# nauful/NLZM

Hardware: AMD Instinct MI355X
Metric: compress MB/s (higher is better)
Workload: dtype u8; 1 GPU; enwik9 stand-in: 1000000000 B stream, -window:28; step = 41 launches of 8 chunks (40136704 B) of the stream; timed: bytes [200683520, 401367040) of 1000000000 (a prefix: the steps asked for end before the stream does); window_bits=28, batch_chunks=8, whole_stream=False

## Files before the change

### nlzm_amd/csrc/nlzm_hip.cpp

```cpp
#include <hip/hip_runtime.h>
#include <dirent.h>
#include <unistd.h>

#include <stdarg.h>
#include <stdint.h>
#include <stdio.h>
#include <stdlib.h>
#include <string.h>

#include <mutex>
#include <vector>

#include "nlzm_host_state.h"
#include "nlzm_report.h"

#include "nlzm_launch.h"

using namespace nlzm;
using namespace nlzm::host;

namespace {

char g_err[kErrText] = "";
std::mutex g_err_mu;
char *thread_err() { return t_dev ? t_dev->err : nullptr; }

int g_hwq_effective = 0;

inline uint32_t clampu(uint32_t v, uint32_t lo, uint32_t hi) { return v < lo ? lo : (v > hi ? hi : v); }

}

namespace nlzm {
int host_error(int code, const char *text)
{
    std::lock_guard<std::mutex> lk(g_err_mu);
    snprintf(g_err, sizeof g_err, "%s", text);
    if (char *te = thread_err()) memcpy(te, g_err, sizeof g_err);
    return code;
}
namespace host {

void error_prefixed(char (&out)[kErrText], const char *text, const char *prefix_fmt, ...)
{
    char prefix[32];
    va_list ap;
    va_start(ap, prefix_fmt);
    vsnprintf(prefix, sizeof prefix, prefix_fmt, ap);
    va_end(ap);
    std::lock_guard<std::mutex> lk(g_err_mu);
    snprintf(out, sizeof out, "%s%.*s", prefix, (int)sizeof out - 32, text ? text : g_err);
}
void error_replace(const char (&text)[kErrText])
{
    std::lock_guard<std::mutex> lk(g_err_mu);
    memcpy(g_err, text, sizeof g_err);
}

DevState g_dev0;
thread_local DevState *t_dev = nullptr;

void free_stream_buffers(Ctx &C)
{
    for (void *p : C.owned) (void)hipFree(p);
    C.owned.clear();
    C.buf = StreamBuffers{}; C.set[0] = C.set[1] = LaunchSet{}; C.set_idx = 0;
    C.open = false;
}
void release_own_io(Ctx &C)
{
    if (C.own_in) { (void)hipFree(C.own_in); C.own_in = nullptr; }
    if (C.own_dst) { (void)hipFree(C.own_dst); C.own_dst = nullptr; }
}
int alloc_own_io(Ctx &C, uint64_t n, uint64_t bound)
{
    release_own_io(C);
    HIPCHK(hipMalloc(&C.own_in, n + 512));
    HIPCHK(hipMalloc(&C.own_dst, bound));
    HIPCHK(hipMemsetAsync(C.own_in + n, 0, 512, C.st));
    return 0;
}

void make_geom(uint64_t n, uint32_t hist_bits_req, Geom &g)
{
    uint32_t hb = hist_bits_req;
    while (hb > 10 && n < (1ull << (hb - 1))) --hb;
    g.n = n;
    g.wbits = hb; g.wmask = (1u << hb) - 1;
    g.frame_bits = clampu(hb - 2, 14, 17);
    g.frame_size = 1u << g.frame_bits;
    g.chunk_size = ((g.frame_size * 15) / 16) - 0x200;
    g.feed = g.chunk_size + kMatchMax + 1;
    g.ht3_shift = 32 - (12 + clampu(hb, 15, 17) - 15);
    g.bt_shift = 32 - (13 + clampu(hb, 16, 20) - 16);
    g.rk_shift = 32 - (15 + clampu(hb, 16, 22) - 16);
    g.tag_mask = (uint32_t)((1ull << (32 - hb)) - 1);
    g.nchunks = (uint32_t)((n + g.chunk_size - 1) / g.chunk_size);
    g.bt_tmask = g.wmask;
}

// ... 2 lines not shown
    uint32_t tb = clampu(g.wbits + 5, 16, 33);
    uint32_t lgn = 1; while ((1ull << lgn) < g.n) lgn++;
    const uint32_t want = lgn + (uint32_t)tbits_per;
    if (want < tb) tb = want < 16 ? 16 : want;
    if ((int64_t)tb > tbits_max) tb = (uint32_t)(tbits_max < 16 ? 16 : tbits_max);
    return tb;
}
bool prefilter_is_bitmap(const Geom &g) { return g.n <= (unsigned long long)g.wmask + 1; }
size_t prefilter_bytes(uint32_t t_bits, bool bitmap)
{
    return bitmap ? (((size_t)1 << t_bits) / 8 < 4 ? (size_t)4 : ((size_t)1 << t_bits) / 8) : (size_t)4 << t_bits;
}
double launch_bytes_per_chunk(const Geom &g) { return 2300.0 * g.chunk_size + 8.0 * g.chunk_size * 4; }

namespace {
int alloc_launch_set(Ctx &C, LaunchSet &S)
{
    const StreamConfig &K = C.cfg;
    const unsigned long long bpos = (unsigned long long)K.batch * C.g.chunk_size;
    DEVALLOC(S.rkhash, K.rkhash_len * 4 + 16);
    DEVALLOC(S.syms, K.batch * K.syms_stride * 4);
    DEVALLOC(S.bits, K.batch * K.bits_stride);
    DEVALLOC(S.fmeta, K.batch * sizeof(FrameMeta));
    DEVALLOC(S.unc, bpos + 16);
    DEVALLOC(S.bt_ready, bpos * 4 * kBtRec);
    DEVALLOC(S.bt_flag, bpos * 4);
    DEVALLOC(S.abort_word, 4);
    DEVALLOC(S.bin_off, (size_t)K.batch * (K.nheads + 1) * 4);
    DEVALLOC(S.bin_pos, bpos * 8);
    if (K.hot_max) {
        DEVALLOC(S.hot_of_bin, (size_t)K.nheads * 4);
        DEVALLOC(S.hot_list, ((size_t)K.hot_max + 1) * 4);
    }
    if (K.in_set) DEVALLOC(S.snap, sizeof(v2::RoundSnap));
    return 0;
}
}

int stream_begin(Ctx &C, const Options &O, const void *d_src, uint64_t n, uint32_t hist_bits_req, void *d_dst, uint64_t dst_cap)
{
    if (!C.inited) return fail(NLZM_HIP_E_NODEVICE, "nlzm_hip_init() has not succeeded");
    if (n >= 0xFFFF0000ull) return fail(NLZM_HIP_E_TOOBIG, "input of %llu bytes needs >32-bit positions", (unsigned long long)n);
    if (hist_bits_req < 10 || hist_bits_req > 28) return fail(NLZM_HIP_E_ARG, "hist_bits %u outside [10,28]", hist_bits_req);
    if (dst_cap < 8) return fail(NLZM_HIP_E_CAPACITY, "dst_cap < 8");
    free_stream_buffers(C);
    make_geom(n, hist_bits_req, C.g);
    const Geom &g = C.g;
    C.d_in = (const uint8_t *)d_src; C.d_dst = (uint8_t *)d_dst; C.dst_cap = dst_cap;
    C.out_pos = 0; C.next_chunk = 0; C.pre_chunk = 0; C.last_launch_ms = 0;
    memset(&C.stats, 0, sizeof C.stats);
    memset(&C.tm, 0, sizeof C.tm);
    C.stats.in_bytes = n;
    StreamConfig &K = C.cfg;
    StreamBuffers &B = C.buf;
    K = StreamConfig{};
    K.in_set = C.pool != nullptr;
    K.batch = (uint32_t)(O.batch < 1 ? 1 : O.batch);
    if (g.nchunks && K.batch > g.nchunks) K.batch = g.nchunks;
    {
        const int64_t room = (int64_t)C.cu_count - (int64_t)pipeline2_role_blocks();
        if (room < 1) return fail(NLZM_HIP_E_ARG, "device has %d CUs: the pipeline needs at least %u", C.cu_count, pipeline2_role_blocks() + 1);
        K.worker_blocks = (uint32_t)(O.worker_blocks > room ? room : (O.worker_blocks < 1 ? 1 : O.worker_blocks));
    }
    K.worker_threads = (uint32_t)O.worker_threads;
    {
        K.nheads = 1u << (32 - g.bt_shift);
        const unsigned long long lanes = (unsigned long long)K.worker_blocks * K.worker_threads;
// ... 12 lines not shown
    K.syms_stride = 3ull * g.chunk_size + 4096;
    K.bits_stride = 2ull * g.chunk_size + 64;
    K.frame_stride = 12 + K.bits_stride + 16 + 2 * K.syms_stride;

    const size_t ht3_bytes = (size_t)8 << (32 - g.ht3_shift), rk_bytes = (size_t)4 << (32 - g.rk_shift), heads_bytes = (size_t)4 << (32 - g.bt_shift);
    {
        const unsigned long long need = (1ull << g.wbits) + (unsigned long long)K.batch * g.chunk_size;
        unsigned long long slots = 1ull << g.wbits;
        while (slots < need) slots <<= 1;
        C.g.bt_tmask = (uint32_t)(slots - 1);
    }
    const size_t tree_bytes = ((size_t)g.bt_tmask + 1) * 8;
    DEVALLOC(B.ht2, 4096 * 4);
    DEVALLOC(B.ht3, ht3_bytes);
    DEVALLOC(B.rk_table, rk_bytes);
    DEVALLOC(B.bt_heads, heads_bytes);
    DEVALLOC(B.bt_tree, tree_bytes);
    DEVALLOC(B.persist, sizeof(Persist));
    DEVFILL(hipMemsetAsync(B.ht2, 0xFF, 4096 * 4, C.st));
    DEVFILL(hipMemsetAsync(B.ht3, 0xFF, ht3_bytes, C.st));
    DEVFILL(hipMemsetAsync(B.rk_table, 0xFF, rk_bytes, C.st));
    DEVFILL(hipMemsetAsync(B.bt_heads, 0xFF, heads_bytes, C.st));
    DEVFILL(hipMemsetAsync(B.bt_tree, 0xFF, tree_bytes, C.st));

    Persist P;
    memset(&P, 0, sizeof P);
    for (uint32_t ctx = 0; ctx < kNumCtx; ctx++) {
        const uint32_t ns = (ctx == kCtxCmd) ? 4 : ((ctx == kCtxLenDirect || ctx >= kCtxSlotHi) ? 8 : 16);
        for (uint32_t i = 0; i <= ns; i++) P.cdf[ctx * kCdfStride + i] = (uint16_t)(i * (16384 / ns));
    }
    for (int i = 0; i < 4; i++) P.rep[i] = (uint32_t)i + 1;
    DEVFILL(hipMemcpyAsync(B.persist, &P, sizeof P, hipMemcpyHostToDevice, C.st));

    if (!K.in_set) {
        size_t free_b = 0, total_b = 0;
        HIPCHK(hipMemGetInfo(&free_b, &total_b));
        const double room = 0.6 * (double)free_b - 4.0 * (double)(1ull << K.t_bits);
        const double per_chunk = launch_bytes_per_chunk(g);
        if (room > per_chunk && (double)K.batch * per_chunk > room) K.batch = (uint32_t)(room / per_chunk);
    }
    const unsigned long long bpos = (unsigned long long)K.batch * g.chunk_size;
    K.rkhash_len = bpos + g.feed + 256 + 1024 + 2048;
    if (K.rkhash_len > n + 2048) K.rkhash_len = n + 2048;
    { uint32_t lg = 1; while ((1ull << lg) < bpos) lg++; K.m_bits = lg + 6 > 28 ? 28 : lg + 6; }
    K.ext_cap = K.pstride < kBtMaxPairs ? (uint32_t)(bpos / 64 + 1024) : 0u;
    if (K.ext_cap && O.block_ext_blocks >= 0) K.ext_cap = (uint32_t)(O.block_ext_blocks < 1 ? 1 : O.block_ext_blocks);

    DEVALLOC(B.scratch, K.batch * K.syms_stride * 4);
    DEVALLOC(B.frames, K.batch * K.frame_stride);
    DEVALLOC(B.dst_off, K.batch * sizeof(unsigned long long));
    for (uint32_t s = 0; s < (K.in_set ? 2u : 1u); s++) { const int rc = alloc_launch_set(C, C.set[s]); if (rc) return rc; }

    for (;;) {
        const int rc_t = dev_alloc(C, &B.pf_T, prefilter_bytes(K.t_bits, K.t_bitmap != 0));
        if (!rc_t) break;
        if (K.in_set || rc_t != NLZM_HIP_E_NOMEM || K.t_bits <= 28) return rc_t;
        (void)hipGetLastError();
        K.t_bits--;
    }
    DEVALLOC(B.pf_M, (size_t)4 << K.m_bits);
    DEVFILL(hipMemsetAsync(B.pf_T, 0, prefilter_bytes(K.t_bits, K.t_bitmap != 0), C.st));
    DEVFILL(hipMemsetAsync(B.pf_M, 0xFF, (size_t)4 << K.m_bits, C.st));
    DEVALLOC(B.pf_h, bpos * 4);
    DEVALLOC(B.pf_h2, bpos * 4);
    DEVALLOC(B.pf_c1, bpos);
    DEVALLOC(B.bt_pairs, bpos * (2ull * K.pstride * 4));
    if (K.ext_cap) DEVALLOC(B.bt_ext, (size_t)K.ext_cap * (2ull * (kBtMaxPairs - K.pstride) * 4));
    DEVALLOC(B.bin_cur, (size_t)K.batch * K.nheads * 4);
    DEVALLOC(B.wcnt, sizeof(WorkerCounters));
    DEVFILL(hipMemsetAsync(B.wcnt, 0, sizeof(WorkerCounters), C.st));
    DEVALLOC(B.bt_undo, (size_t)K.nheads * worker_undo_bytes_per_lane());
    if (K.hot_max) DEVALLOC(B.hot_undo, (size_t)K.hot_max * worker_hot_undo_bytes_per_wave());

    DEVALLOC(B.v2_ft, (size_t)v2::kFtRing * v2::kFtStride * 4);
    DEVALLOC(B.v2_tp, (size_t)v2::kTpRing * v2::kTpStride * 4);
    DEVALLOC(B.v2_tf, (size_t)v2::kTpRing * v2::kTfStride * 4);
    DEVALLOC(B.v2_state, sizeof(v2::StateV2));
    DEVALLOC(B.v2_hx, sizeof(v2::Hx));
    if (K.helper) DEVALLOC(B.v2_hb, v2::kHelpers * sizeof(v2::HelpBox));
    DEVFILL(hipMemsetAsync(B.v2_state, 0, sizeof(v2::StateV2), C.st));
    C.v2_launch_no = 0;

    const uint8_t hdr[4] = { (uint8_t)(g.wbits >> 8), (uint8_t)g.wbits, (uint8_t)(g.frame_bits >> 8), (uint8_t)g.frame_bits };
    DEVFILL(hipMemcpyAsync(C.d_dst, hdr, 4, hipMemcpyHostToDevice, C.st));
    C.out_pos = 4;

    if (C.pool && C.pool->measuring) return 0;
    HIPCHK(hipStreamSynchronize(C.st));
    C.open = true;
    return 0;
}

int step_pre(Ctx &C, uint32_t todo, StepPlan &P, bool ahead)
{
    const Geom &g = C.g;
    const StreamConfig &K = C.cfg;
    const StreamBuffers &B = C.buf;
    if (ahead) { if (!K.in_set) return fail(NLZM_HIP_E_ARG, "no second launch set"); C.set_idx ^= 1; }
    const LaunchSet &L = C.set[C.set_idx];
    const uint32_t c0 = C.pre_chunk, nb = todo < K.batch ? todo : K.batch, c1 = c0 + nb;
    C.pre_chunk = c1;
    P.c0 = c0; P.c1 = c1; P.nb = nb;
    P.set = C.set_idx; P.ahead = ahead;
    hipEvent_t *ev = C.ev[P.set];
    Globals &G = P.G;
    memset(&G, 0, sizeof G);
    G.in = C.d_in; G.rkhash = nullptr; G.ht2 = B.ht2; G.ht3 = B.ht3; G.rk_table = B.rk_table;
    G.bt_heads = B.bt_heads; G.bt_tree = B.bt_tree; G.persist = B.persist;
    G.syms = L.syms; G.syms_stride = K.syms_stride; G.bits = L.bits; G.bits_stride = K.bits_stride;
    G.fmeta = L.fmeta; G.chunk0 = c0;
    G.cap_words = C.stage.cap_words; G.cap_cap = C.stage.cap_cap; G.cap_lo = C.stage.cap_lo; G.cap_hi = C.stage.cap_hi; G.cap_used = C.stage.cap_used;
    G.workers = 1;
    const unsigned long long a0 = (unsigned long long)c0 * g.chunk_size;
    unsigned long long a1 = (unsigned long long)c1 * g.chunk_size;
    if (a1 > g.n) a1 = g.n;
    G.batch_a0 = (uint32_t)a0;
    {
        const unsigned long long lo = a0 > 1024 ? a0 - 1024 : 0;
        unsigned long long hi = a1 + g.feed + 256;
        if (hi + 255 > g.n) hi = g.n >= 255 ? g.n - 255 : 0;
        HIPCHK(hipEventRecord(ev[kEvRkBegin], C.st));
        if (hi > lo && hi - lo > K.rkhash_len) return fail(NLZM_HIP_E_ARG, "launch of %u chunks is larger than the stream was opened for", nb);
        G.rkhash = L.rkhash - lo;
        if (g.n >= 256 && hi > lo) launch_rk_hash(C.d_in, g.n, lo, hi, L.rkhash - lo, C.st);
    }
    HIPCHK(hipEventRecord(ev[kEvRkEnd], C.st));
    {
        const unsigned long long cnt = a1 - a0;
        G.bt_ready = L.bt_ready; G.bt_pairs = B.bt_pairs; G.bt_flag = L.bt_flag; G.unc = L.unc;
        G.bt_pstride = K.pstride; G.bt_ext = B.bt_ext; G.bt_ext_cap = K.ext_cap; G.bt_ext_cur = &B.v2_hx->ext_cur;
        G.bin_off = L.bin_off; G.bin_pos = L.bin_pos; G.nheads = K.nheads; G.wthreads = K.worker_threads;
        G.abort_word = L.abort_word; G.wcnt = B.wcnt; G.bt_undo = B.bt_undo;
        HIPCHK(hipMemsetAsync(L.bt_ready, 0, cnt * 4 * kBtRec, C.st));
        HIPCHK(hipMemsetAsync(L.bt_flag, 0, cnt * 4, C.st));
        HIPCHK(hipMemsetAsync(L.abort_word, 0, 4, C.st));
        HIPCHK(hipMemsetAsync(L.bin_off, 0, (size_t)nb * (K.nheads + 1) * 4, C.st));
        launch_prefilter(C.d_in, g.n, (uint32_t)a0, (uint32_t)a1, g.wmask, K.t_bits, K.t_bitmap, K.m_bits, B.pf_T, B.pf_M, B.pf_h, B.pf_h2,
                         B.pf_c1, L.unc, C.st);
        launch_bin(C.d_in, g, c0, nb, K.nheads, L.bin_off, B.bin_cur, L.bin_pos, L.unc, (uint32_t)a0, C.st);
        if (K.hot_max) {
            const unsigned long long lpos = (unsigned long long)K.batch * g.chunk_size;
            const double by_pace = K.in_set ? (double)lpos / 480.0 : (C.last_launch_ms > 0 ? 24.0 * C.last_launch_ms : (double)lpos / 240.0);
            const uint32_t hot_min = K.hot_min > 0 ? K.hot_min : (uint32_t)(by_pace < 512 ? 512 : (by_pace > 1e9 ? 1e9 : by_pace));
            launch_hot_select(L.bin_off, nb, K.nheads, K.hot_max, hot_min, L.hot_of_bin, L.hot_list, B.wcnt, C.st);
            G.hot_of_bin = L.hot_of_bin; G.hot_list = L.hot_list; G.hot_undo = B.hot_undo;
        }
    }
    {
        v2::Hx &h = C.hx_host;
        memset(&h, 0, sizeof h);
        h.f_pos = h.t_pos = h.t_out = h.p_pos = (uint32_t)a0;
        h.p_seg = ((unsigned long long)(uint32_t)a0 << 32) | (uint32_t)a0;
        if (!ahead) HIPCHK(hipMemcpyAsync(B.v2_hx, &h, sizeof h, hipMemcpyHostToDevice, C.st));
        P.V.ft = B.v2_ft; P.V.tp = B.v2_tp; P.V.tf = B.v2_tf; P.V.hx = B.v2_hx; P.V.state = B.v2_state; P.V.hb = B.v2_hb;
        G.progress = &B.v2_hx->f_pos;
        G.test_fail = K.test_fail_launch >= 0 && (int64_t)C.v2_launch_no == K.test_fail_launch ? 1u : 0u;
        G.table_shape = K.table_shape; G.launch_par = (uint32_t)(C.v2_launch_no++ & 1u);
    }
    HIPCHK(hipEventRecord(ev[kEvPrepEnd], C.st));
    return 0;
}

int step_post_issue(Ctx &C, const StepPlan &P)
{
    const StreamConfig &K = C.cfg;
    const LaunchSet &L = C.set[P.set];
    hipEvent_t *ev = C.ev[P.set];
    const uint32_t nb = P.nb;
    C.post_hm.resize(nb); C.post_hoff.resize(nb);
    C.post_aborted = 0;
    HIPCHK(hipEventRecord(ev[kEvLaunchEnd], C.st));
    launch_rans(L.syms, K.syms_stride, L.bits, K.bits_stride, L.fmeta, C.buf.scratch, K.syms_stride, C.buf.frames,
                K.frame_stride, (uint32_t)K.frame_stride, nb, C.st);
    HIPCHK(hipEventRecord(ev[kEvCoderEnd], C.st));
    HIPCHK(hipMemcpyAsync(C.post_hm.data(), L.fmeta, nb * sizeof(FrameMeta), hipMemcpyDeviceToHost, C.st));
    if (P.ahead) {
        HIPCHK(hipMemcpyAsync(&C.post_snap, L.snap, sizeof(v2::RoundSnap), hipMemcpyDeviceToHost, C.st));
        return 0;
    }
    HIPCHK(hipMemcpyAsync(&C.post_P, C.buf.persist, sizeof C.post_P, hipMemcpyDeviceToHost, C.st));
    HIPCHK(hipMemcpyAsync(&C.post_aborted, L.abort_word, 4, hipMemcpyDeviceToHost, C.st));
    HIPCHK(hipMemcpyAsync(&C.hx_host, C.buf.v2_hx, sizeof(v2::Hx), hipMemcpyDeviceToHost, C.st));
    return 0;
}
int step_post_check(Ctx &C, const StepPlan &P)
{
    const Geom &g = C.g;
    const StreamConfig &K = C.cfg;
    const LaunchSet &L = C.set[P.set];
    hipEvent_t *ev = C.ev[P.set];
    const uint32_t c0 = P.c0, c1 = P.c1, nb = P.nb;
    std::vector<FrameMeta> &hm = C.post_hm;
    std::vector<unsigned long long> &hoff = C.post_hoff;
    HIPCHK(hipStreamSynchronize(C.st));
    HIPCHK(hipGetLastError());
    if (P.ahead) { C.post_P.error = C.post_snap.error; C.post_P.next_chunk = C.post_snap.next_chunk; C.post_aborted = C.post_snap.aborted; C.hx_host = C.post_snap.hx; }
    const Persist &Pst = C.post_P;
    const uint32_t aborted = C.post_aborted;
    float rk_ms = 0, pre_ms = 0;
    HIPCHK(hipEventElapsedTime(&rk_ms, ev[kEvRkBegin], ev[kEvRkEnd]));
    HIPCHK(hipEventElapsedTime(&pre_ms, ev[kEvRkEnd], ev[kEvPrepEnd]));
    C.tm.prep_ms += rk_ms + pre_ms; C.tm.prep_launches += 5; C.tm.total_ms += rk_ms + pre_ms;
    C.arena_out = false;
    if (Pst.error || C.hx_host.err) {
        const v2::Hx &h = C.hx_host;
        WorkerCounters wc{};
        (void)hipMemcpy(&wc, C.buf.wcnt, sizeof wc, hipMemcpyDeviceToHost);
        char where[kErrText];
        stage_error_text(where, sizeof where, h, wc);
        return fail(NLZM_HIP_E_KERNEL, "device error %u in chunks [%u,%u) (parser stopped at chunk %u): %s", Pst.error ? Pst.error : h.err, c0, c1, Pst.next_chunk, where);
    }
    C.arena_out = K.ext_cap && C.hx_host.ext_cur > K.ext_cap;
    if (C.arena_out) return fail(NLZM_HIP_E_KERNEL, "the extension arena of the BT4 pair lists (%u blocks per launch) was used up in chunks [%u,%u): more positions with over %u "
                                     "record-setters than a block set reserves for", K.ext_cap, c0, c1, K.pstride);
    if (aborted) return fail(NLZM_HIP_E_KERNEL, "worker lanes aborted (code %u) in chunks [%u,%u)", aborted, c0, c1);
    if (Pst.next_chunk != c1) return fail(NLZM_HIP_E_KERNEL, "master stopped at chunk %u, expected %u", Pst.next_chunk, c1);
    unsigned long long pos = C.out_pos;
    for (uint32_t f = 0; f < nb; f++) {
        const uint32_t room = g.frame_size - ((c0 + f) == 0 ? 4 : 0);
        if (hm[f].out_len > room)
            return fail(NLZM_HIP_E_KERNEL, "frame %u is %u bytes: the reference would assert (:610)", c0 + f, hm[f].out_len);
        hoff[f] = pos; pos += hm[f].out_len;
    }
    if (pos + 4 > C.dst_cap) return fail(NLZM_HIP_E_CAPACITY, "dst_cap %llu too small", (unsigned long long)C.dst_cap);
    if (StageCapture &S = C.stage; S.want_frame >= (int64_t)c0 && S.want_frame < (int64_t)c1) {
        const uint32_t f = (uint32_t)(S.want_frame - c0);
        S.got_meta = hm[f];
        S.got_syms.resize(hm[f].nsyms); S.got_bits.resize(hm[f].nbits_bytes);
        HIPCHK(hipMemcpy(S.got_syms.data(), L.syms + f * K.syms_stride, hm[f].nsyms * 4ull, hipMemcpyDeviceToHost));
        HIPCHK(hipMemcpy(S.got_bits.data(), L.bits + f * K.bits_stride, hm[f].nbits_bytes, hipMemcpyDeviceToHost));
        S.got = true;
    }
    HIPCHK(hipMemcpyAsync(C.buf.dst_off, hoff.data(), nb * sizeof(unsigned long long), hipMemcpyHostToDevice, C.st));
    HIPCHK(hipEventRecord(ev[kEvGatherBegin], C.st));
    launch_gather(C.buf.frames, K.frame_stride, C.buf.dst_off, L.fmeta, C.d_dst, nb, C.st);
    HIPCHK(hipEventRecord(ev[kEvGatherEnd], C.st));
    C.post_pos = pos;
    return 0;
}
int step_post_done(Ctx &C, const StepPlan &P, float pipe_ms)
{
    hipEvent_t *ev = C.ev[P.set];
    const unsigned long long pos = C.post_pos;
    const uint32_t c1 = P.c1;
    HIPCHK(hipStreamSynchronize(C.st));
    float a = pipe_ms, b = 0, c = 0;
    if (pipe_ms < 0) HIPCHK(hipEventElapsedTime(&a, ev[kEvLaunchBegin], ev[kEvLaunchEnd]));
    HIPCHK(hipEventElapsedTime(&b, ev[kEvLaunchEnd], ev[kEvCoderEnd]));
    HIPCHK(hipEventElapsedTime(&c, ev[kEvGatherBegin], ev[kEvGatherEnd]));
    C.tm.match_parse_ms += a; C.tm.match_parse_launches++;
    if (a > 0) C.last_launch_ms = a;
    C.tm.rans_ms += b + c; C.tm.rans_launches++;
    C.tm.total_ms += a + b + c;
    C.out_pos = pos;
    C.next_chunk = c1;
    return 0;
}
namespace {
int step_post(Ctx &C, const StepPlan &P, float pipe_ms)
{
    int rc = step_post_issue(C, P);
    if (!rc) rc = step_post_check(C, P);
    if (!rc) rc = step_post_done(C, P, pipe_ms);
    return rc;
}
}

int stream_step(Ctx &C, uint32_t max_chunks, uint64_t *in_done, uint64_t *out_done, int *finished)
{
    if (!C.open) return fail(NLZM_HIP_E_ARG, "no open stream");
    const Geom &g = C.g;
    uint32_t todo = g.nchunks - C.next_chunk;
    if (max_chunks && todo > max_chunks) todo = max_chunks;
    while (todo) {
        StepPlan P;
        int rc = step_pre(C, todo, P);
        if (rc) return rc;
        HIPCHK(hipEventRecord(C.ev[P.set][kEvLaunchBegin], C.st));
        launch_pipeline2(g, P.G, P.V, P.c0, P.c1, C.cfg.worker_blocks, C.st);
        rc = step_post(C, P, -1.0f);
        if (rc) return rc;
        todo -= P.nb;
    }
    if (in_done) {
        const unsigned long long d = (unsigned long long)C.next_chunk * g.chunk_size;
        *in_done = d < g.n ? d : g.n;
    }
    if (out_done) *out_done = C.out_pos;
    if (finished) *finished = C.next_chunk >= g.nchunks;
    return 0;
}

namespace {
int refresh_stats(Ctx &C, bool report)
{
    Persist P;
    HIPCHK(hipMemcpy(&P, C.buf.persist, sizeof P, hipMemcpyDeviceToHost));
    nlzm_hip_stats &s = C.stats;
    s.out_bytes = C.out_pos;
    s.bt_calls = P.cnt.bt_calls; s.bt_tests = P.cnt.bt_tests; s.cmp_bytes = P.cnt.cmp_bytes; s.ht_rows = P.cnt.ht_rows;
    s.rk_probes = P.cnt.rk_probes; s.rk_inserts = P.cnt.rk_inserts; s.positions = P.cnt.positions;
    s.nice_positions = P.cnt.nice_positions; s.segments = P.cnt.segments; s.n_literal = P.cnt.n_literal;
    s.n_dict = P.cnt.n_dict; s.n_rep = P.cnt.n_rep; s.rans_syms = P.cnt.rans_syms; s.bit_ops = P.cnt.bit_ops;
    s.frames = P.cnt.frames; s.shifts = P.cnt.shifts; s.uncertain_positions = P.cnt.uncertain_positions;
    memcpy(C.prof_last, P.prof, sizeof C.prof_last);
    acct_figures(P, C.acct);
    if (report) stage_report(stderr, P);
    WorkerCounters wc;
    HIPCHK(hipMemcpy(&wc, C.buf.wcnt, sizeof wc, hipMemcpyDeviceToHost));
    s.bt_calls += wc.bt_calls; s.bt_tests += wc.bt_tests; s.cmp_bytes += wc.cmp_bytes;
    C.wc_last = wc;
    if (report) worker_report(stderr, wc, C.cfg.hot_max != 0);
    return 0;
}
}
// ... 17 lines not shown
    Ctx &C = D.ctx;
    static std::once_flag hwq_once;
    std::call_once(hwq_once, [] {
        const char *have = getenv("GPU_MAX_HW_QUEUES");
        if (have && *have) { g_hwq_effective = atoi(have); return; }
        bool kfd = false;
        if (DIR *d = opendir("/proc/self/fd")) {
            while (struct dirent *e = readdir(d)) {
                char path[64], to[64];
                snprintf(path, sizeof path, "/proc/self/fd/%s", e->d_name);
                const ssize_t k = readlink(path, to, sizeof to - 1);
                if (k > 0) { to[k] = 0; if (!strcmp(to, "/dev/kfd")) kfd = true; }
            }
            closedir(d);
        }
        if (kfd) { g_hwq_effective = 4; return; }
        (void)setenv("GPU_MAX_HW_QUEUES", "16", 0);
        g_hwq_effective = 16;
    });
    int ndev = 0;
    hipError_t e = hipGetDeviceCount(&ndev);
    if (e != hipSuccess || ndev <= 0) return fail(NLZM_HIP_E_NODEVICE, "no HIP device (%s)", hipGetErrorString(e));
    if (device < 0 || device >= ndev) return fail(NLZM_HIP_E_ARG, "device %d out of range (%d present)", device, ndev);
    HIPCHK(hipSetDevice(device));
    hipDeviceProp_t prop;
    HIPCHK(hipGetDeviceProperties(&prop, device));
    if (strncmp(prop.gcnArchName, "gfx950", 6) != 0)
        return fail(NLZM_HIP_E_NODEVICE, "device %d is %s; this library is built for gfx950 only", device, prop.gcnArchName);
    if (C.inited && C.device == device) return 0;
    if (C.inited) dev_shutdown(D);
    C.device = device;
    C.cu_count = prop.multiProcessorCount;
    HIPCHK(hipStreamCreateWithFlags(&C.st, hipStreamNonBlocking));
    for (auto &ev : C.ev[0]) HIPCHK(hipEventCreate(&ev));
    C.inited = true;
    return 0;
}

void dev_shutdown(DevState &D)
{
    Ctx &C = D.ctx;
    if (!C.inited) return;
    blocks_close(D, true);
    feed_close(D);
    free_stream_buffers(C);
    release_own_io(C);
    if (C.stage.cap_words) { (void)hipFree(C.stage.cap_words); C.stage.cap_words = nullptr; }
    if (C.stage.cap_used) { (void)hipFree(C.stage.cap_used); C.stage.cap_used = nullptr; }
    for (auto &ev : C.ev[0]) if (ev) { (void)hipEventDestroy(ev); ev = nullptr; }
    if (C.st) { (void)hipStreamDestroy(C.st); C.st = nullptr; }
    C.inited = false;
}

}

int host_stream(hipStream_t *st)
{
    Ctx &C = cur().ctx;
    if (!C.inited) return fail(NLZM_HIP_E_NODEVICE, "nlzm_hip_init() has not succeeded (no device: there is no CPU fallback)");
    *st = C.st;
    return 0;
}
void host_decode_setup(int64_t *ring_option, int *cu_count)
{
    const DevState &D = cur();
    *ring_option = D.opt.decode_ring; *cu_count = D.ctx.cu_count;
}
}

extern "C" {

int nlzm_hip_init(int device) { return dev_init(cur(), device); }
void nlzm_hip_shutdown(void) { dev_shutdown(cur()); }

const char *nlzm_hip_last_error(void) { return g_err; }

uint64_t nlzm_hip_compress_bound(uint64_t n)
{
    return 16 + 131072 + (n / 14848 + 1) * 16384;
}

void nlzm_hip_geometry(uint64_t flen, uint32_t hist_bits_req, uint32_t *hist_bits, uint32_t *frame_bits,
// ... 161 lines not shown
```

### nlzm_amd/csrc/nlzm_hip_blocks.cpp

```cpp
#include <stdio.h>
#include <string.h>

#include <algorithm>
#include <array>
#include <chrono>
#include <mutex>
#include <thread>
#include <vector>

#include "nlzm_host_state.h"
#include "nlzm_container_plan.h"
#include "nlzm_launch.h"
#include "nlzm_report.h"

using namespace nlzm;
using namespace nlzm::host;

namespace {

int block_ctx_init(Ctx &c, const Ctx &of)
{
    c.device = of.device; c.cu_count = of.cu_count;
    HIPCHK(hipStreamCreateWithFlags(&c.st, hipStreamNonBlocking));
    for (auto &set : c.ev) for (auto &ev : set) HIPCHK(hipEventCreate(&ev));
    c.inited = true;
    return 0;
}
void block_ctx_destroy(Ctx &c)
{
    free_stream_buffers(c);
    for (auto &set : c.ev) for (auto &ev : set) if (ev) { (void)hipEventDestroy(ev); ev = nullptr; }
    if (c.st) { (void)hipStreamDestroy(c.st); c.st = nullptr; }
    c.inited = false;
}

Options block_stream_options(const Options &S, int64_t worker_blocks, int64_t batch, int64_t tbits_max, uint32_t index)
{
    Options o = S;
    o.report = 0;
    o.worker_blocks = worker_blocks; o.batch = batch; o.tbits_max = tbits_max;
    o.worker_threads = S.block_threads;
    o.hot_waves = S.block_hot_waves;
    o.helper = S.block_helper;
    o.test_fail_launch = (int64_t)index == S.test_fail_stream ? S.test_fail_launch : -1;
    return o;
}

}

uint32_t host::blocks_capacity(const DevState &D)
{
    if (!D.ctx.inited) return 0;
    const int64_t roles_live = (int64_t)pipeline2_role_blocks() - (D.opt.block_helper ? 0 : (int64_t)v2::kHelpers);
    const int64_t cap = D.ctx.cu_count / (roles_live + 1);
    return (uint32_t)(cap < 0 ? 0 : cap > 64 ? 64 : cap);
}

bool host::idle_block_pool_dropped()
{
    DevState &D = cur();
    if (!D.jobs.empty() || !D.blocks_pool) return false;
    (void)hipFree(D.blocks_pool);
    D.blocks_pool = nullptr; D.blocks_pool_size = 0;
    return true;
// ... 131 lines not shown
            D.group_ev.push_back(ev);
        }
        return 0;
    }();
    if (rc) blocks_close(D);
    return rc;
}

static int blocks_step_impl(DevState &D, uint32_t max_chunks_per_block, uint64_t *in_done_total, int *finished, double *device_ms)
{
    Ctx &C = D.ctx;
    const size_t nj = D.jobs.size();
    hipEvent_t e0 = C.ev[0][kEvCallBegin], e1 = C.ev[0][kEvCallEnd];
    HIPCHK(hipEventRecord(e0, C.st));
    HIPCHK(hipStreamSynchronize(C.st));
    if (nj > stream2_pack_capacity()) return fail(NLZM_HIP_E_ARG, "too many streams for one launch");
    DevState::Rounds &R = D.rounds;
    hipStream_t gs = D.group_st[0];
    for (auto &p : R.plan) if (p.size() != nj) p.assign(nj, StepPlan{});
    const uint32_t kAll = 0xFFFFFFFFu;
    std::vector<uint32_t> quota(nj, max_chunks_per_block ? max_chunks_per_block : kAll);
    auto queue_round = [&](uint32_t q, bool in_call) -> int {
        std::vector<uint32_t> &act = R.act[q];
        act.clear();
        std::vector<uint32_t> todo(nj, 0);
        for (size_t i = 0; i < nj; i++) {
            const Ctx &c = D.jobs[i].c;
            const uint32_t rem = c.g.nchunks - c.pre_chunk;
            const uint32_t want = in_call ? quota[i] : (max_chunks_per_block ? max_chunks_per_block : kAll);
            todo[i] = rem < want ? rem : want;
            if (todo[i]) act.push_back((uint32_t)i);
        }
        if (act.empty()) return 0;
        for (uint32_t i : act) { const int rc = step_pre(D.jobs[i].c, todo[i], R.plan[q][i], true); if (rc) return rc; }
        uint8_t *ph = (uint8_t *)D.pack_host + (size_t)q * stream2_pack_size(), *pd = (uint8_t *)D.pack_dev + (size_t)q * stream2_pack_size();
        for (uint32_t k = 0; k < act.size(); k++) {
            Ctx &c = D.jobs[act[k]].c;
            const StepPlan &P = R.plan[q][act[k]];
            HIPCHK(hipStreamWaitEvent(gs, c.ev[P.set][kEvPrepEnd], 0));
            fill_stream2_args(ph, k, c.g, P.G, P.V, P.c0, P.c1, c.set[P.set].snap);
        }
        HIPCHK(hipMemcpyAsync(pd, ph, stream2_pack_size(), hipMemcpyHostToDevice, gs));
        launch_round_open(pd, (uint32_t)act.size(), gs);
        HIPCHK(hipEventRecord(D.group_ev[q][0], gs));
        launch_pipeline2_multi(pd, (uint32_t)act.size(), (uint32_t)D.blocks_wb, gs);
        HIPCHK(hipEventRecord(D.group_ev[q][1], gs));
        launch_round_close(pd, (uint32_t)act.size(), gs);
        HIPCHK(hipEventRecord(D.group_ev[q][2], gs));
        return 0;
    };
    if (!R.have) {
        const int rc = queue_round(R.q, true);
        if (rc) return rc;
        R.have = !R.act[R.q].empty();
    }
    while (R.have) {
        const uint32_t q = R.q;
        bool more = false;
        for (uint32_t i : R.act[q]) { const uint32_t nb = R.plan[q][i].nb; if (quota[i] != kAll) quota[i] -= nb < quota[i] ? nb : quota[i]; }
        for (size_t i = 0; i < nj; i++) more |= quota[i] && D.jobs[i].c.pre_chunk < D.jobs[i].c.g.nchunks;
        { const int rc = queue_round(q ^ 1, more); if (rc) return rc; }
        {
            int first_rc = 0;
            char first_msg[kErrText] = "";
            std::vector<int> rcs(nj, 0);
            auto note = [&](uint32_t i, int rc) {
                if (rc && !rcs[i]) rcs[i] = rc;
// ... 209 lines not shown
```

### nlzm_amd/csrc/nlzm_host_state.h

```cpp
#pragma once

#include "nlzm_host_util.h"

#include <array>
#include <vector>

#include "nlzm_core.h"
#include "nlzm_v2.h"

namespace nlzm {
namespace host {

struct Pool {
    uint8_t *base = nullptr;
    size_t size = 0, used = 0;
    bool measuring = false;
};

struct Options {
    int64_t batch = 32;
    int64_t worker_blocks = 240;
    int64_t worker_threads = 128;
    int64_t hot_waves = 2;
    int64_t hot_min = 0;
    int64_t tbits_max = 34;
    int64_t block_threads = 320;
    int64_t block_hot_waves = 3;
    int64_t block_batch = 8;
    int64_t tbits_per = 4;
    int64_t keep_pool = 1;
    int64_t helper = 1;
    int64_t block_helper = 0;
    int64_t multi_same = 0;
    int64_t table_shape = 0;
    int64_t test_fail_launch = -1;
    int64_t test_fail_stream = 0;
    int64_t block_ext_blocks = -1;
    int64_t report = 0;
    int64_t container_set_blocks = 32;
    int64_t decode_ring = 0;
};

struct StreamConfig {
    bool in_set = false;
    uint32_t batch = 0;
    uint32_t worker_blocks = 0, worker_threads = 0;
    uint32_t nheads = 0;
    uint32_t hot_max = 0;
    uint32_t hot_min = 0;
    uint32_t t_bits = 0, m_bits = 0;
    uint32_t t_bitmap = 0;
    uint32_t pstride = kBtMaxPairs, ext_cap = 0;
    bool helper = false;
    uint32_t table_shape = 0;
    int64_t test_fail_launch = -1;
    unsigned long long rkhash_len = 0;
    unsigned long long syms_stride = 0, bits_stride = 0, frame_stride = 0;
};

struct LaunchSet {
    uint32_t *rkhash = nullptr, *bt_ready = nullptr, *bt_flag = nullptr, *abort_word = nullptr, *bin_off = nullptr, *bin_pos = nullptr,
             *hot_of_bin = nullptr, *hot_list = nullptr, *syms = nullptr;
    uint8_t *unc = nullptr, *bits = nullptr;
    FrameMeta *fmeta = nullptr;
    v2::RoundSnap *snap = nullptr;
};

struct StreamBuffers {
    uint32_t *ht2 = nullptr, *ht3 = nullptr, *rk_table = nullptr, *bt_heads = nullptr, *bt_tree = nullptr;
    Persist *persist = nullptr;
    uint32_t *scratch = nullptr;
    uint8_t *frames = nullptr;
    unsigned long long *dst_off = nullptr;
    uint32_t *pf_T = nullptr, *pf_M = nullptr, *pf_h = nullptr, *pf_h2 = nullptr; uint8_t *pf_c1 = nullptr;
    uint32_t *bt_pairs = nullptr, *bt_ext = nullptr;
    uint32_t *bin_cur = nullptr, *bt_undo = nullptr;
    unsigned long long *hot_undo = nullptr;
    WorkerCounters *wcnt = nullptr;
    uint32_t *v2_ft = nullptr, *v2_tp = nullptr, *v2_tf = nullptr, *v2_state = nullptr;
    v2::Hx *v2_hx = nullptr;
    v2::HelpBox *v2_hb = nullptr;
};

enum { kEvLaunchBegin, kEvLaunchEnd , kEvCoderEnd, kEvGatherBegin, kEvGatherEnd, kEvRkBegin, kEvRkEnd , kEvPrepEnd,
       kEvCallBegin, kEvCallEnd, kEvN };

struct StageCapture {
    uint32_t *cap_words = nullptr; unsigned long long cap_cap = 0, cap_lo = 0, cap_hi = 0; unsigned long long *cap_used = nullptr;
    int64_t want_frame = -1;
    std::vector<uint32_t> got_syms; std::vector<uint8_t> got_bits; FrameMeta got_meta{};
    bool got = false;
};
struct Ctx {
    bool inited = false;
    int device = 0, cu_count = 0;
    hipStream_t st = nullptr;
    hipEvent_t ev[2][kEvN] = {};
    Pool *pool = nullptr;

    bool open = false;
    StreamConfig cfg;
    Geom g{};
    const uint8_t *d_in = nullptr;
    uint8_t *d_dst = nullptr;
    uint64_t dst_cap = 0, out_pos = 0;
    uint32_t next_chunk = 0;
    uint32_t pre_chunk = 0;
    uint32_t v2_launch_no = 0;

    StreamBuffers buf;
    LaunchSet set[2];
    uint32_t set_idx = 0;
    std::vector<void *> owned;
    uint8_t *own_in = nullptr, *own_dst = nullptr;

    StageCapture stage;

    v2::Hx hx_host;
    std::vector<FrameMeta> post_hm; std::vector<unsigned long long> post_hoff; Persist post_P; uint32_t post_aborted = 0; unsigned long long post_pos = 0;
    v2::RoundSnap post_snap;
    double last_launch_ms = 0;
    bool arena_out = false;
    nlzm_hip_stats stats{};
    nlzm_hip_timing tm{};
    unsigned long long prof_last[kPfSlots] = {};
    WorkerCounters wc_last{};
    double acct[8] = {};
};

bool idle_block_pool_dropped();

template <class T> int dev_alloc(Ctx &C, T **p, size_t bytes)
{
    if (!C.pool) {
        hipError_t e = hipMalloc((void **)p, bytes);
        if (e == hipErrorOutOfMemory && idle_block_pool_dropped()) {
            (void)hipGetLastError();
            e = hipMalloc((void **)p, bytes);
        }
        if (e != hipSuccess) return fail(e == hipErrorOutOfMemory ? NLZM_HIP_E_NOMEM : NLZM_HIP_E_NODEVICE, "hipMalloc of %zu bytes failed: %s", bytes, hipGetErrorString(e));
        C.owned.push_back(*p);
        return 0;
    }
    Pool &P = *C.pool;
    const size_t at = (P.used + 255) & ~(size_t)255;
    if (!P.measuring && at + bytes > P.size) return fail(NLZM_HIP_E_NOMEM, "stream pool of %zu bytes is too small", P.size);
    *p = P.measuring ? nullptr : (T *)(P.base + at);
    P.used = at + bytes;
    return 0;
}
#define DEVALLOC(ptr, bytes) do { const int rc_ = dev_alloc(C, &(ptr), (bytes)); if (rc_) return rc_; } while (0)
#define DEVFILL(expr) do { if (!(C.pool && C.pool->measuring)) HIPCHK(expr); } while (0)

struct StepPlan {
    uint32_t c0 = 0, c1 = 0, nb = 0; Globals G; v2::GlobalsV2 V;
    uint32_t set = 0;
    bool ahead = false;
};

struct BlockJob {
    Ctx c;
    uint64_t lo = 0, n = 0, len = 0, bound = 0;
    uint8_t *d_out = nullptr;
    int rc = 0;
    bool redo = false;
    Pool pool;
};

struct DevState {
    char err[kErrText] = "";
    Ctx ctx;
    Options opt;
    std::vector<BlockJob> jobs;
    uint8_t *blocks_pool = nullptr;
    size_t blocks_pool_size = 0;
    std::vector<hipStream_t> group_st;
    std::vector<std::array<hipEvent_t, 3>> group_ev;
    void *pack_host = nullptr, *pack_dev = nullptr;
    uint64_t blocks_n = 0;
    const uint8_t *blocks_src = nullptr;
    uint32_t blocks_hist = 0;
    int64_t blocks_wb = 0;
    uint64_t blocks_per = 0;
    uint64_t redo_streams = 0;
    uint64_t container_sets = 0;
    struct Rounds {
        bool have = false;
        uint32_t q = 0;
        std::vector<StepPlan> plan[2];
        std::vector<uint32_t> act[2];
    } rounds;
    struct Feed {
        bool open = false, finished = false;
        uint64_t n = 0, fed = 0, arrived = 0, taken = 0;
        uint8_t *pin[2] = { nullptr, nullptr };
        hipEvent_t ev[2] = { nullptr, nullptr };
        uint64_t end_of[2] = { 0, 0 };
        hipStream_t st = nullptr;
        uint32_t next = 0;
    } feed;
};
extern DevState g_dev0;
extern thread_local DevState *t_dev;
inline DevState &cur() { return t_dev ? *t_dev : g_dev0; }

static_assert(sizeof(nlzm_hip_stats) % sizeof(uint64_t) == 0 && alignof(nlzm_hip_stats) == alignof(uint64_t), "nlzm_hip_stats is uint64_t counters and nothing else: they are added up as an array");
inline void add_stats(nlzm_hip_stats &to, const nlzm_hip_stats &from)
{
    uint64_t *d = (uint64_t *)&to; const uint64_t *s = (const uint64_t *)&from;
    for (size_t k = 0; k < sizeof(nlzm_hip_stats) / sizeof(uint64_t); k++) d[k] += s[k];
}

void error_prefixed(char (&out)[kErrText], const char *text, const char *prefix_fmt, ...);
void error_replace(const char (&text)[kErrText]);

int dev_init(DevState &D, int device);
void dev_shutdown(DevState &D);
void make_geom(uint64_t n, uint32_t hist_bits_req, Geom &g);
uint32_t prefilter_tbits(const Geom &g, int64_t tbits_per, int64_t tbits_max);
bool prefilter_is_bitmap(const Geom &g);
size_t prefilter_bytes(uint32_t t_bits, bool bitmap);
double launch_bytes_per_chunk(const Geom &g);
int stream_begin(Ctx &C, const Options &O, const void *d_src, uint64_t n, uint32_t hist_bits_req, void *d_dst, uint64_t dst_cap);
int step_pre(Ctx &C, uint32_t todo, StepPlan &P, bool ahead = false);
int step_post_issue(Ctx &C, const StepPlan &P);
int step_post_check(Ctx &C, const StepPlan &P);
int step_post_done(Ctx &C, const StepPlan &P, float pipe_ms);
int stream_step(Ctx &C, uint32_t max_chunks, uint64_t *in_done, uint64_t *out_done, int *finished);
int stream_finish(Ctx &C, uint64_t *dst_len, bool report);
void free_stream_buffers(Ctx &C);
int alloc_own_io(Ctx &C, uint64_t n, uint64_t bound);
void release_own_io(Ctx &C);
void blocks_close(DevState &D, bool drop_pool = false);
uint32_t blocks_capacity(const DevState &D);
void feed_close(DevState &D);

}
}
```

Before: 6.867 MB/s.

## Double-buffer single-stream steps with a high-priority launch stream overlapping prep and post

Single-stream compression now allocates two launch sets when memory allows and runs the main pipeline kernel on a separate high-priority stream. The next batch's prefilter and binning on the main stream can then overlap the current batch's match/parse launch. Post-processing reads one round snapshot instead of several separate device-to-host copies of persist, abort word and Hx state. In exchange it uses more device memory for the second launch set and adds event-based cross-stream synchronisation, and the hot-bin selection now happens on the launch stream.

```diff
diff --git a/nlzm_amd/csrc/nlzm_hip.cpp b/nlzm_amd/csrc/nlzm_hip.cpp
--- a/nlzm_amd/csrc/nlzm_hip.cpp
+++ b/nlzm_amd/csrc/nlzm_hip.cpp
@@ -13,6 +13,7 @@
 
 #include "nlzm_host_state.h"
 #include "nlzm_report.h"
+#include "nlzm_stream_plan.h"
 
 #include "nlzm_launch.h"
 
@@ -66,6 +67,25 @@
     C.owned.clear();
     C.buf = StreamBuffers{}; C.set[0] = C.set[1] = LaunchSet{}; C.set_idx = 0;
     C.open = false;
+}
+void release_launch_stream(Ctx &C)
+{
+    for (auto &set : C.launch_ev) for (auto &ev : set) if (ev) { (void)hipEventDestroy(ev); ev = nullptr; }
+    if (C.launch_st) { (void)hipStreamDestroy(C.launch_st); C.launch_st = nullptr; }
+    if (C.launch_pack) { (void)hipHostFree(C.launch_pack); C.launch_pack = nullptr; }
+}
+namespace {
+size_t pack_entry_bytes() { return (size_t)(stream2_pack_size() / stream2_pack_capacity()); }
+int make_launch_stream(Ctx &C)
+{
+    if (C.launch_st) return 0;
+    int lo_p = 0, hi_p = 0;
+    HIPCHK(hipDeviceGetStreamPriorityRange(&lo_p, &hi_p));
+    HIPCHK(hipStreamCreateWithPriority(&C.launch_st, hipStreamNonBlocking, hi_p));
+    for (auto &set : C.launch_ev) for (auto &ev : set) HIPCHK(hipEventCreate(&ev));
+    HIPCHK(hipHostMalloc(&C.launch_pack, 2 * pack_entry_bytes(), hipHostMallocDefault));
+    return 0;
+}
 }
 void release_own_io(Ctx &C)
 {
@@ -134,7 +154,7 @@
         DEVALLOC(S.hot_of_bin, (size_t)K.nheads * 4);
         DEVALLOC(S.hot_list, ((size_t)K.hot_max + 1) * 4);
     }
-    if (K.in_set) DEVALLOC(S.snap, sizeof(v2::RoundSnap));
+    DEVALLOC(S.snap, sizeof(v2::RoundSnap));
     return 0;
 }
 }
@@ -213,12 +233,15 @@
     for (int i = 0; i < 4; i++) P.rep[i] = (uint32_t)i + 1;
     DEVFILL(hipMemcpyAsync(B.persist, &P, sizeof P, hipMemcpyHostToDevice, C.st));
 
+    K.depth = 2;
     if (!K.in_set) {
         size_t free_b = 0, total_b = 0;
         HIPCHK(hipMemGetInfo(&free_b, &total_b));
-        const double room = 0.6 * (double)free_b - 4.0 * (double)(1ull << K.t_bits);
-        const double per_chunk = launch_bytes_per_chunk(g);
-        if (room > per_chunk && (double)K.batch * per_chunk > room) K.batch = (uint32_t)(room / per_chunk);
+        const stream_plan::Plan plan = stream_plan::make_plan((double)free_b, 4.0 * (double)(1ull << K.t_bits) ,
+                                                              launch_bytes_per_chunk(g), K.batch, g.nchunks);
+        K.batch = plan.batch; K.depth = plan.depth;
+        const int rc = make_launch_stream(C);
+        if (rc) return rc;
     }
     const unsigned long long bpos = (unsigned long long)K.batch * g.chunk_size;
     K.rkhash_len = bpos + g.feed + 256 + 1024 + 2048;
@@ -230,7 +253,7 @@
     DEVALLOC(B.scratch, K.batch * K.syms_stride * 4);
     DEVALLOC(B.frames, K.batch * K.frame_stride);
     DEVALLOC(B.dst_off, K.batch * sizeof(unsigned long long));
-    for (uint32_t s = 0; s < (K.in_set ? 2u : 1u); s++) { const int rc = alloc_launch_set(C, C.set[s]); if (rc) return rc; }
+    for (uint32_t s = 0; s < K.depth; s++) { const int rc = alloc_launch_set(C, C.set[s]); if (rc) return rc; }
 
     for (;;) {
         const int rc_t = dev_alloc(C, &B.pf_T, prefilter_bytes(K.t_bits, K.t_bitmap != 0));
@@ -272,17 +295,27 @@
     return 0;
 }
 
-int step_pre(Ctx &C, uint32_t todo, StepPlan &P, bool ahead)
+static void select_hot_bins(Ctx &C, const StepPlan &P, hipStream_t st)
+{
+    const StreamConfig &K = C.cfg;
+    const LaunchSet &L = C.set[P.set];
+    const unsigned long long lpos = (unsigned long long)K.batch * C.g.chunk_size;
+    const double by_pace = K.in_set ? (double)lpos / 480.0 : (C.last_launch_ms > 0 ? 24.0 * C.last_launch_ms : (double)lpos / 240.0);
+    const uint32_t hot_min = K.hot_min > 0 ? K.hot_min : (uint32_t)(by_pace < 512 ? 512 : (by_pace > 1e9 ? 1e9 : by_pace));
+    launch_hot_select(L.bin_off, P.nb, K.nheads, K.hot_max, hot_min, L.hot_of_bin, L.hot_list, C.buf.wcnt, st);
+}
+
+int step_pre(Ctx &C, uint32_t todo, StepPlan &P)
 {
     const Geom &g = C.g;
     const StreamConfig &K = C.cfg;
     const StreamBuffers &B = C.buf;
-    if (ahead) { if (!K.in_set) return fail(NLZM_HIP_E_ARG, "no second launch set"); C.set_idx ^= 1; }
+    if (K.depth > 1) C.set_idx ^= 1;
     const LaunchSet &L = C.set[C.set_idx];
     const uint32_t c0 = C.pre_chunk, nb = todo < K.batch ? todo : K.batch, c1 = c0 + nb;
     C.pre_chunk = c1;
     P.c0 = c0; P.c1 = c1; P.nb = nb;
-    P.set = C.set_idx; P.ahead = ahead;
+    P.set = C.set_idx;
     hipEvent_t *ev = C.ev[P.set];
     Globals &G = P.G;
     memset(&G, 0, sizeof G);
@@ -320,19 +353,11 @@
                          B.pf_c1, L.unc, C.st);
         launch_bin(C.d_in, g, c0, nb, K.nheads, L.bin_off, B.bin_cur, L.bin_pos, L.unc, (uint32_t)a0, C.st);
         if (K.hot_max) {
-            const unsigned long long lpos = (unsigned long long)K.batch * g.chunk_size;
-            const double by_pace = K.in_set ? (double)lpos / 480.0 : (C.last_launch_ms > 0 ? 24.0 * C.last_launch_ms : (double)lpos / 240.0);
-            const uint32_t hot_min = K.hot_min > 0 ? K.hot_min : (uint32_t)(by_pace < 512 ? 512 : (by_pace > 1e9 ? 1e9 : by_pace));
-            launch_hot_select(L.bin_off, nb, K.nheads, K.hot_max, hot_min, L.hot_of_bin, L.hot_list, B.wcnt, C.st);
+            if (K.in_set) select_hot_bins(C, P, C.st);
             G.hot_of_bin = L.hot_of_bin; G.hot_list = L.hot_list; G.hot_undo = B.hot_undo;
         }
     }
     {
-        v2::Hx &h = C.hx_host;
-        memset(&h, 0, sizeof h);
-        h.f_pos = h.t_pos = h.t_out = h.p_pos = (uint32_t)a0;
-        h.p_seg = ((unsigned long long)(uint32_t)a0 << 32) | (uint32_t)a0;
-        if (!ahead) HIPCHK(hipMemcpyAsync(B.v2_hx, &h, sizeof h, hipMemcpyHostToDevice, C.st));
         P.V.ft = B.v2_ft; P.V.tp = B.v2_tp; P.V.tf = B.v2_tf; P.V.hx = B.v2_hx; P.V.state = B.v2_state; P.V.hb = B.v2_hb;
         G.progress = &B.v2_hx->f_pos;
         G.test_fail = K.test_fail_launch >= 0 && (int64_t)C.v2_launch_no == K.test_fail_launch ? 1u : 0u;
@@ -349,19 +374,12 @@
     hipEvent_t *ev = C.ev[P.set];
     const uint32_t nb = P.nb;
     C.post_hm.resize(nb); C.post_hoff.resize(nb);
-    C.post_aborted = 0;
     HIPCHK(hipEventRecord(ev[kEvLaunchEnd], C.st));
     launch_rans(L.syms, K.syms_stride, L.bits, K.bits_stride, L.fmeta, C.buf.scratch, K.syms_stride, C.buf.frames,
                 K.frame_stride, (uint32_t)K.frame_stride, nb, C.st);
     HIPCHK(hipEventRecord(ev[kEvCoderEnd], C.st));
     HIPCHK(hipMemcpyAsync(C.post_hm.data(), L.fmeta, nb * sizeof(FrameMeta), hipMemcpyDeviceToHost, C.st));
-    if (P.ahead) {
-        HIPCHK(hipMemcpyAsync(&C.post_snap, L.snap, sizeof(v2::RoundSnap), hipMemcpyDeviceToHost, C.st));
-        return 0;
-    }
-    HIPCHK(hipMemcpyAsync(&C.post_P, C.buf.persist, sizeof C.post_P, hipMemcpyDeviceToHost, C.st));
-    HIPCHK(hipMemcpyAsync(&C.post_aborted, L.abort_word, 4, hipMemcpyDeviceToHost, C.st));
-    HIPCHK(hipMemcpyAsync(&C.hx_host, C.buf.v2_hx, sizeof(v2::Hx), hipMemcpyDeviceToHost, C.st));
+    HIPCHK(hipMemcpyAsync(&C.post_snap, L.snap, sizeof(v2::RoundSnap), hipMemcpyDeviceToHost, C.st));
     return 0;
 }
 int step_post_check(Ctx &C, const StepPlan &P)
@@ -375,23 +393,22 @@
     std::vector<unsigned long long> &hoff = C.post_hoff;
     HIPCHK(hipStreamSynchronize(C.st));
     HIPCHK(hipGetLastError());
-    if (P.ahead) { C.post_P.error = C.post_snap.error; C.post_P.next_chunk = C.post_snap.next_chunk; C.post_aborted = C.post_snap.aborted; C.hx_host = C.post_snap.hx; }
-    const Persist &Pst = C.post_P;
-    const uint32_t aborted = C.post_aborted;
+    const v2::RoundSnap &Pst = C.post_snap;
+    const v2::Hx &h = Pst.hx;
+    const uint32_t aborted = Pst.aborted;
     float rk_ms = 0, pre_ms = 0;
     HIPCHK(hipEventElapsedTime(&rk_ms, ev[kEvRkBegin], ev[kEvRkEnd]));
     HIPCHK(hipEventElapsedTime(&pre_ms, ev[kEvRkEnd], ev[kEvPrepEnd]));
     C.tm.prep_ms += rk_ms + pre_ms; C.tm.prep_launches += 5; C.tm.total_ms += rk_ms + pre_ms;
     C.arena_out = false;
-    if (Pst.error || C.hx_host.err) {
-        const v2::Hx &h = C.hx_host;
+    if (Pst.error || h.err) {
         WorkerCounters wc{};
         (void)hipMemcpy(&wc, C.buf.wcnt, sizeof wc, hipMemcpyDeviceToHost);
         char where[kErrText];
         stage_error_text(where, sizeof where, h, wc);
         return fail(NLZM_HIP_E_KERNEL, "device error %u in chunks [%u,%u) (parser stopped at chunk %u): %s", Pst.error ? Pst.error : h.err, c0, c1, Pst.next_chunk, where);
     }
-    C.arena_out = K.ext_cap && C.hx_host.ext_cur > K.ext_cap;
+    C.arena_out = K.ext_cap && h.ext_cur > K.ext_cap;
     if (C.arena_out) return fail(NLZM_HIP_E_KERNEL, "the extension arena of the BT4 pair lists (%u blocks per launch) was used up in chunks [%u,%u): more positions with over %u "
                                      "record-setters than a block set reserves for", K.ext_cap, c0, c1, K.pstride);
     if (aborted) return fail(NLZM_HIP_E_KERNEL, "worker lanes aborted (code %u) in chunks [%u,%u)", aborted, c0, c1);
@@ -426,7 +443,6 @@
     const uint32_t c1 = P.c1;
     HIPCHK(hipStreamSynchronize(C.st));
     float a = pipe_ms, b = 0, c = 0;
-    if (pipe_ms < 0) HIPCHK(hipEventElapsedTime(&a, ev[kEvLaunchBegin], ev[kEvLaunchEnd]));
     HIPCHK(hipEventElapsedTime(&b, ev[kEvLaunchEnd], ev[kEvCoderEnd]));
     HIPCHK(hipEventElapsedTime(&c, ev[kEvGatherBegin], ev[kEvGatherEnd]));
     C.tm.match_parse_ms += a; C.tm.match_parse_launches++;
@@ -437,31 +453,61 @@
     C.next_chunk = c1;
     return 0;
 }
-namespace {
-int step_post(Ctx &C, const StepPlan &P, float pipe_ms)
-{
-    int rc = step_post_issue(C, P);
-    if (!rc) rc = step_post_check(C, P);
-    if (!rc) rc = step_post_done(C, P, pipe_ms);
-    return rc;
-}
-}
-
 int stream_step(Ctx &C, uint32_t max_chunks, uint64_t *in_done, uint64_t *out_done, int *finished)
 {
     if (!C.open) return fail(NLZM_HIP_E_ARG, "no open stream");
+    if (!C.launch_st) return fail(NLZM_HIP_E_ARG, "the stream has no launch stream (a stream of a block set steps with its set)");
     const Geom &g = C.g;
     uint32_t todo = g.nchunks - C.next_chunk;
     if (max_chunks && todo > max_chunks) todo = max_chunks;
-    while (todo) {
-        StepPlan P;
-        int rc = step_pre(C, todo, P);
-        if (rc) return rc;
-        HIPCHK(hipEventRecord(C.ev[P.set][kEvLaunchBegin], C.st));
-        launch_pipeline2(g, P.G, P.V, P.c0, P.c1, C.cfg.worker_blocks, C.st);
-        rc = step_post(C, P, -1.0f);
-        if (rc) return rc;
-        todo -= P.nb;
+    StepPlan plan[2];
+    uint32_t head = 0, prepped = 0, launched = 0;
+    auto prepare = [&](StepPlan &P) -> int {
+        const int rc = step_pre(C, todo, P);
+        if (!rc) todo -= P.nb;
+        return rc;
+    };
+    auto launch = [&](const StepPlan &P) -> int {
+        hipEvent_t *lev = C.launch_ev[P.set];
+        void *pack = (uint8_t *)C.launch_pack + P.set * pack_entry_bytes();
+        fill_stream2_args(pack, 0, g, P.G, P.V, P.c0, P.c1, C.set[P.set].snap);
+        HIPCHK(hipStreamWaitEvent(C.launch_st, C.ev[P.set][kEvPrepEnd], 0));
+        if (C.cfg.hot_max) select_hot_bins(C, P, C.launch_st);
+        launch_round_open(pack, 1, C.launch_st);
+        HIPCHK(hipEventRecord(lev[0], C.launch_st));
+        launch_pipeline2(g, P.G, P.V, P.c0, P.c1, C.cfg.worker_blocks, C.launch_st);
+        HIPCHK(hipEventRecord(lev[1], C.launch_st));
+        launch_round_close(pack, 1, C.launch_st);
+        HIPCHK(hipEventRecord(lev[2], C.launch_st));
+        return 0;
+    };
+    auto ended = [&](const StepPlan &P, float &ms) -> int {
+        hipEvent_t *lev = C.launch_ev[P.set];
+        HIPCHK(hipEventSynchronize(lev[1]));
+        HIPCHK(hipEventElapsedTime(&ms, lev[0], lev[1]));
+        if (ms > 0) C.last_launch_ms = ms;
+        return 0;
+    };
+    auto collect = [&](const StepPlan &P) -> int {
+        HIPCHK(hipStreamWaitEvent(C.st, C.launch_ev[P.set][2], 0));
+        int rc = step_post_issue(C, P);
+        if (!rc) rc = step_post_check(C, P);
+        float ms = 0;
+        if (!rc) rc = ended(P, ms);
+        return rc ? rc : step_post_done(C, P, ms);
+    };
+    int rc = 0;
+    while (!rc && (todo || prepped)) {
+        while (!rc && todo && prepped < C.cfg.depth) { rc = prepare(plan[(head + prepped) & 1]); if (!rc) prepped++; }
+        if (!rc && !launched) { rc = launch(plan[head & 1]); launched = 1; }
+        if (!rc && prepped > 1) { float ms = 0; rc = ended(plan[head & 1], ms); if (!rc) rc = launch(plan[(head + 1) & 1]); launched = 2; }
+        if (!rc) { rc = collect(plan[head & 1]); head++; prepped--; launched--; }
+    }
+    if (rc) {
+        (void)hipStreamSynchronize(C.launch_st);
+        (void)hipStreamSynchronize(C.st);
+        (void)hipGetLastError();
+        return rc;
     }
     if (in_done) {
         const unsigned long long d = (unsigned long long)C.next_chunk * g.chunk_size;
@@ -545,7 +591,7 @@
     C.device = device;
     C.cu_count = prop.multiProcessorCount;
     HIPCHK(hipStreamCreateWithFlags(&C.st, hipStreamNonBlocking));
-    for (auto &ev : C.ev[0]) HIPCHK(hipEventCreate(&ev));
+    for (auto &set : C.ev) for (auto &ev : set) HIPCHK(hipEventCreate(&ev));
     C.inited = true;
     return 0;
 }
@@ -560,7 +606,8 @@
     release_own_io(C);
     if (C.stage.cap_words) { (void)hipFree(C.stage.cap_words); C.stage.cap_words = nullptr; }
     if (C.stage.cap_used) { (void)hipFree(C.stage.cap_used); C.stage.cap_used = nullptr; }
-    for (auto &ev : C.ev[0]) if (ev) { (void)hipEventDestroy(ev); ev = nullptr; }
+    for (auto &set : C.ev) for (auto &ev : set) if (ev) { (void)hipEventDestroy(ev); ev = nullptr; }
+    release_launch_stream(C);
     if (C.st) { (void)hipStreamDestroy(C.st); C.st = nullptr; }
     C.inited = false;
 }
diff --git a/nlzm_amd/csrc/nlzm_hip_blocks.cpp b/nlzm_amd/csrc/nlzm_hip_blocks.cpp
--- a/nlzm_amd/csrc/nlzm_hip_blocks.cpp
+++ b/nlzm_amd/csrc/nlzm_hip_blocks.cpp
@@ -30,6 +30,7 @@
 {
     free_stream_buffers(c);
     for (auto &set : c.ev) for (auto &ev : set) if (ev) { (void)hipEventDestroy(ev); ev = nullptr; }
+    release_launch_stream(c);
     if (c.st) { (void)hipStreamDestroy(c.st); c.st = nullptr; }
     c.inited = false;
 }
@@ -227,7 +228,7 @@
             if (todo[i]) act.push_back((uint32_t)i);
         }
         if (act.empty()) return 0;
-        for (uint32_t i : act) { const int rc = step_pre(D.jobs[i].c, todo[i], R.plan[q][i], true); if (rc) return rc; }
+        for (uint32_t i : act) { const int rc = step_pre(D.jobs[i].c, todo[i], R.plan[q][i]); if (rc) return rc; }
         uint8_t *ph = (uint8_t *)D.pack_host + (size_t)q * stream2_pack_size(), *pd = (uint8_t *)D.pack_dev + (size_t)q * stream2_pack_size();
         for (uint32_t k = 0; k < act.size(); k++) {
             Ctx &c = D.jobs[act[k]].c;
diff --git a/nlzm_amd/csrc/nlzm_host_state.h b/nlzm_amd/csrc/nlzm_host_state.h
--- a/nlzm_amd/csrc/nlzm_host_state.h
+++ b/nlzm_amd/csrc/nlzm_host_state.h
@@ -44,6 +44,7 @@
 struct StreamConfig {
     bool in_set = false;
     uint32_t batch = 0;
+    uint32_t depth = 1;
     uint32_t worker_blocks = 0, worker_threads = 0;
     uint32_t nheads = 0;
     uint32_t hot_max = 0;
@@ -82,7 +83,7 @@
     v2::HelpBox *v2_hb = nullptr;
 };
 
-enum { kEvLaunchBegin, kEvLaunchEnd , kEvCoderEnd, kEvGatherBegin, kEvGatherEnd, kEvRkBegin, kEvRkEnd , kEvPrepEnd,
+enum { kEvLaunchEnd , kEvCoderEnd, kEvGatherBegin, kEvGatherEnd, kEvRkBegin, kEvRkEnd , kEvPrepEnd,
        kEvCallBegin, kEvCallEnd, kEvN };
 
 struct StageCapture {
@@ -96,6 +97,9 @@
     int device = 0, cu_count = 0;
     hipStream_t st = nullptr;
     hipEvent_t ev[2][kEvN] = {};
+    hipStream_t launch_st = nullptr;
+    hipEvent_t launch_ev[2][3] = {};
+    void *launch_pack = nullptr;
     Pool *pool = nullptr;
 
     bool open = false;
@@ -116,8 +120,7 @@
 
     StageCapture stage;
 
-    v2::Hx hx_host;
-    std::vector<FrameMeta> post_hm; std::vector<unsigned long long> post_hoff; Persist post_P; uint32_t post_aborted = 0; unsigned long long post_pos = 0;
+    std::vector<FrameMeta> post_hm; std::vector<unsigned long long> post_hoff; unsigned long long post_pos = 0;
     v2::RoundSnap post_snap;
     double last_launch_ms = 0;
     bool arena_out = false;
@@ -155,7 +158,6 @@
 struct StepPlan {
     uint32_t c0 = 0, c1 = 0, nb = 0; Globals G; v2::GlobalsV2 V;
     uint32_t set = 0;
-    bool ahead = false;
 };
 
 struct BlockJob {
@@ -222,13 +224,14 @@
 size_t prefilter_bytes(uint32_t t_bits, bool bitmap);
 double launch_bytes_per_chunk(const Geom &g);
 int stream_begin(Ctx &C, const Options &O, const void *d_src, uint64_t n, uint32_t hist_bits_req, void *d_dst, uint64_t dst_cap);
-int step_pre(Ctx &C, uint32_t todo, StepPlan &P, bool ahead = false);
+int step_pre(Ctx &C, uint32_t todo, StepPlan &P);
 int step_post_issue(Ctx &C, const StepPlan &P);
 int step_post_check(Ctx &C, const StepPlan &P);
 int step_post_done(Ctx &C, const StepPlan &P, float pipe_ms);
 int stream_step(Ctx &C, uint32_t max_chunks, uint64_t *in_done, uint64_t *out_done, int *finished);
 int stream_finish(Ctx &C, uint64_t *dst_len, bool report);
 void free_stream_buffers(Ctx &C);
+void release_launch_stream(Ctx &C);
 int alloc_own_io(Ctx &C, uint64_t n, uint64_t bound);
 void release_own_io(Ctx &C);
 void blocks_close(DevState &D, bool drop_pool = false);
diff --git a/nlzm_amd/csrc/nlzm_stream_plan.h b/nlzm_amd/csrc/nlzm_stream_plan.h
--- /dev/null
+++ b/nlzm_amd/csrc/nlzm_stream_plan.h
@@ -0,0 +1,25 @@
+#pragma once
+
+#include <stdint.h>
+
+namespace nlzm {
+namespace stream_plan {
+
+struct Plan {
+    uint32_t batch = 0;
+    uint32_t depth = 1;
+};
+
+inline Plan make_plan(double free_bytes, double table_bytes, double per_chunk, uint32_t batch, uint32_t nchunks)
+{
+    Plan P;
+    P.batch = batch < 1 ? 1u : batch;
+    const double room = 0.6 * free_bytes - table_bytes;
+    const bool cut = room > per_chunk && (double)P.batch * per_chunk > room;
+    if (cut) P.batch = (uint32_t)(room / per_chunk);
+    P.depth = !cut && nchunks > P.batch && 2.0 * (double)P.batch * per_chunk <= room ? 2u : 1u;
+    return P;
+}
+
+}
+}
```

Measured after the change: 7.003 MB/s (median of 6 runs). +2.0%, better.
